# Q-Minh/point-cloud-processing

Measured on AMD Instinct MI355X. Metric: kNN+normal-estimation Mqueries/s (k=15), higher is better.
Workload: dtype f32

## Files before the change

point-cloud-processing_amd/build.py:

```python
import os
import subprocess
import sys

HERE = os.path.dirname(os.path.abspath(__file__))
CSRC = os.path.join(HERE, "csrc")
INCLUDE = os.path.join(os.path.dirname(HERE), "include")
OBJ_DIR = os.path.join(HERE, "_obj")
LIB = os.path.join(HERE, "libpcpx.so")
SOURCES = ["pcpx_query.hip", "pcpx_few.hip", "pcpx_range.hip", "pcpx_cluster.hip", "pcpx_segment.hip", "pcpx_subsample.hip", "pcpx_keypoints.hip", "pcpx_descriptors.hip", "pcpx_match.hip", "pcpx_register.hip", "pcpx_icp.hip", "pcpx_planes.hip", "pcpx_voxel.hip", "pcpx_mls.hip", "pcpx_filter.hip", "pcpx_normals.hip", "pcpx_prep.hip", "pcpx_orient.hip", "pcpx_build.hip", "pcpx_shard.hip", "pcpx_sort.hip",
           "pcpx_comm.hip", "pcpx_kd.hip", "pcpx_isosurface.hip", "pcpx_simplify.hip", "pcpx_runtime.hip", "pcpx_api.hip"]
HEADERS = [os.path.join(CSRC, "pcpx_internal.h"), os.path.join(CSRC, "pcpx_device.h"), os.path.join(CSRC, "pcpx_box_bound.h"), os.path.join(CSRC, "pcpx_eig3.h"), os.path.join(CSRC, "pcpx_curve.h"),
           os.path.join(CSRC, "pcpx_curve_table.h"), os.path.join(CSRC, "pcpx_scan.h"), os.path.join(CSRC, "pcpx_unionfind.h"), os.path.join(CSRC, "pcpx_labels.h"), os.path.join(CSRC, "pcpx_keep.h"), os.path.join(CSRC, "pcpx_stage.h"), os.path.join(CSRC, "pcpx_lease.h"), os.path.join(CSRC, "pcpx_horn.h"), os.path.join(CSRC, "pcpx_plane_solve.h"), os.path.join(CSRC, "pcpx_ransac.h"), os.path.join(CSRC, "pcpx_fixed_sum.h"), os.path.join(CSRC, "pcpx_plane_fit.h"),
           os.path.join(INCLUDE, "pcpx.h"), os.path.join(INCLUDE, "pcpx_radius.h"), os.path.join(INCLUDE, "pcpx_cluster.h"),
           os.path.join(INCLUDE, "pcpx_subsample.h"), os.path.join(INCLUDE, "pcpx_segment.h"), os.path.join(INCLUDE, "pcpx_features.h"),
           os.path.join(INCLUDE, "pcpx_keypoints.h"), os.path.join(INCLUDE, "pcpx_descriptors.h"), os.path.join(INCLUDE, "pcpx_match.h"),
           os.path.join(INCLUDE, "pcpx_register.h"), os.path.join(INCLUDE, "pcpx_icp.h"), os.path.join(INCLUDE, "pcpx_planes.h"), os.path.join(INCLUDE, "pcpx_voxel.h"), os.path.join(INCLUDE, "pcpx_mls.h")]
ARCH = "gfx950"
FLAGS = ["-O3", "-std=c++17", "-fPIC", "-ffp-contract=off", "-fno-slp-vectorize", "--offload-arch=" + ARCH,
         "-Wall", "-Werror=uninitialized", "-Werror=inline-asm", "-I" + INCLUDE]


def _hipcc():
    for c in (os.environ.get("HIPCC"), "/opt/rocm/bin/hipcc", "hipcc"):
        if c and (os.path.isabs(c) and os.path.exists(c) or not os.path.isabs(c)):
            return c
    return "hipcc"


def _stale(target, deps):
    if not os.path.exists(target):
        return True
    t = os.path.getmtime(target)
    return any(os.path.getmtime(d) > t for d in deps)


def build(force=False, verbose=False, extra_flags=(), tag=""):
    obj_dir = OBJ_DIR + ("_" + tag if tag else "")
    lib = LIB if not tag else os.path.join(HERE, "libpcpx_%s.so" % tag)
    os.makedirs(obj_dir, exist_ok=True)
    objs = []
    hipcc = _hipcc()
    for src in SOURCES:
        s = os.path.join(CSRC, src)
        o = os.path.join(obj_dir, src.replace(".hip", ".o"))
        objs.append(o)
        if force or _stale(o, [s] + HEADERS):
            cmd = [hipcc] + FLAGS + list(extra_flags) + ["-c", s, "-o", o]
            if verbose:
                print(" ".join(cmd), flush=True)
            subprocess.check_call(cmd)
    if force or _stale(lib, objs):
        cmd = [hipcc, "--offload-arch=" + ARCH, "-shared", "-fPIC", "-o", lib] + objs + ["-ldl", "-Wl,-rpath,/opt/rocm/lib"]
        if verbose:
            print(" ".join(cmd), flush=True)
        subprocess.check_call(cmd)
    return lib


if __name__ == "__main__":
    print(build(force="--force" in sys.argv, verbose=True))
```

point-cloud-processing_amd/csrc/pcpx_box_bound.h:

```cpp
#ifndef PCPX_BOX_BOUND_H
#define PCPX_BOX_BOUND_H

#include <cfloat>
#include <cmath>

#if defined(__HIPCC__)
#define PCPX_BOX_BOUND_FN __host__ __device__ inline __attribute__((always_inline))
#else
#define PCPX_BOX_BOUND_FN inline
#endif

namespace pcpx {

template <class Box>
PCPX_BOX_BOUND_FN float box_bound_fused(const Box& b, float qx, float qy, float qz)
{
    const float dx = fmaxf(fmaxf(b.lo(0) - qx, qx - b.hi(0)), 0.f);
    const float dy = fmaxf(fmaxf(b.lo(1) - qy, qy - b.hi(1)), 0.f);
    const float dz = fmaxf(fmaxf(b.lo(2) - qz, qz - b.hi(2)), 0.f);
    return __builtin_fmaf(dz, dz, __builtin_fmaf(dy, dy, __builtin_fmaf(dx, dx, b.poison)));
}

constexpr float BOX_BOUND_K = 1.f + 0x1p-20f;

PCPX_BOX_BOUND_FN float box_bound_tau(float tau) { return tau * BOX_BOUND_K + FLT_MIN; }

}

#undef PCPX_BOX_BOUND_FN
#endif
```

point-cloud-processing_amd/csrc/pcpx_device.h:

```cpp
#ifndef PCPX_DEVICE_H
#define PCPX_DEVICE_H

#include "pcpx_internal.h"

#include <cmath>
#include <limits>
#include <type_traits>

#pragma clang fp contract(off)

namespace pcpx {
namespace {

constexpr int WAVES_PER_BLOCK = 1;

__device__ __forceinline__ u32 wave_in_block() { return __builtin_amdgcn_readfirstlane(threadIdx.x >> 6); }

__device__ __forceinline__ u32 virtual_block()
{
    u32 per = gridDim.x >> 3;
    return (blockIdx.x & 7u) * per + (blockIdx.x >> 3);
}

__device__ __forceinline__ float sq3(float dx, float dy, float dz) { return dx * dx + dy * dy + dz * dz; }

typedef float float_pair __attribute__((ext_vector_type(2)));
__device__ __forceinline__ float box_d2(const NodeBox& b, float qx, float qy, float qz)
{
    float dx = fmaxf(fmaxf(b.lo(0) - qx, qx - b.hi(0)), 0.f);
    float dy = fmaxf(fmaxf(b.lo(1) - qy, qy - b.hi(1)), 0.f);
    float dz = fmaxf(fmaxf(b.lo(2) - qz, qz - b.hi(2)), 0.f);
    return sq3(dx, dy, dz) + b.poison;
}

struct NodeBox4 {
    NodeBox c[W];
};

struct Normals8 {
    float x[LEAF];
    float y[LEAF];
    float z[LEAF];
};
static_assert(sizeof(Normals8) == 12 * LEAF, "normal record must be dense");

__device__ __forceinline__ NodeBox4 load_node4(const NodeBox* first_child)
{
    typedef u32 u32x16 __attribute__((ext_vector_type(16)));
    u32x16 a, b;
    const u64 address = reinterpret_cast<uintptr_t>(first_child);
    const u32 address_lo = __builtin_amdgcn_readfirstlane(static_cast<u32>(address));
    const u32 address_hi = __builtin_amdgcn_readfirstlane(static_cast<u32>(address >> 32));
    const u64 uniform = (static_cast<u64>(address_hi) << 32) | address_lo;
    asm volatile("s_load_dwordx16 %0, %2, 0x0\n\ts_load_dwordx16 %1, %2, 0x40\n\ts_waitcnt lgkmcnt(0)"
                 : "=&s"(a), "=&s"(b)
                 : "s"(uniform));
    NodeBox4 out;
    u32* o = reinterpret_cast<u32*>(&out);
#pragma unroll
    for (int i = 0; i < 16; ++i) {
        o[i] = a[i];
        o[16 + i] = b[i];
    }
    return out;
}

__host__ __device__ __forceinline__ u32 fmix32(u32 x)
{
    x ^= x >> 16;
    x *= 0x85EBCA6Bu;
    x ^= x >> 13;
    x *= 0xC2B2AE35u;
    x ^= x >> 16;
    return x;
}

__device__ __forceinline__ bool any_lane(bool c) { return __builtin_amdgcn_ballot_w64(c) != 0ull; }

template <class T>
__device__ __forceinline__ T load_const(const T* p)
{
    static_assert(sizeof(T) % 4 == 0, "record size");
    typedef const __attribute__((address_space(4))) u32* const_u32_ptr;
    const_u32_ptr c = (const_u32_ptr)(reinterpret_cast<uintptr_t>(p));
    T out;
    u32* o = reinterpret_cast<u32*>(&out);
#pragma unroll
    for (unsigned i = 0; i < sizeof(T) / 4; ++i) o[i] = c[i];
    return out;
}

__device__ __forceinline__ u32 lds_address(const void* p)
{
    return static_cast<u32>(reinterpret_cast<uintptr_t>(p));
}


template <bool X16, bool KEEP = false>
struct WalkerT {
    u64 pend;
    u32 ploc;
    int l;
    u32 l2;
    u32 lshift0;
    u64 leaf_need[W];

    static __device__ __forceinline__ u32 level_base(int d) { return 0x55555555u >> (32 - 2 * d); }

    template <class Need>
    __device__ __forceinline__ u32 child_mask(const TreeView& t, int d, u32 loc, Need&& need)
    {
        return child_mask_at(t, level_base(d + 1) + (loc << LOGW), need);
    }
    template <class Need>
    __device__ __forceinline__ u32 child_mask_at(const TreeView& t, u32 first_child, Need&& need)
    {
        const NodeBox4 cb = X16 ? load_node4(t.nodes + first_child) : load_const(reinterpret_cast<const NodeBox4*>(t.nodes + first_child));
        u32 m;
#pragma unroll
        for (int c = W - 1; c >= 0; --c) {
            const u64 lanes = __builtin_amdgcn_ballot_w64(need(cb.c[c]));
            if (KEEP) leaf_need[c] = lanes;
            if (c == W - 1) asm("s_cmp_lg_u64 %1, 0\n\ts_cselect_b32 %0, 1, 0" : "=s"(m) : "s"(lanes) : "scc");
            else asm("s_cmp_lg_u64 %1, 0\n\ts_addc_u32 %0, %0, %0" : "+s"(m) : "s"(lanes) : "scc");
        }
        return m;
    }

    template <class Need>
    __device__ __forceinline__ bool start(const TreeView& t, Need&& need, u32& n_expand)
    {
        pend = 0;
        ploc = 0;
        l = 0;
        l2 = 0;
        lshift0 = static_cast<u32>(30 - 2 * t.depth);
        asm("" : "+s"(lshift0));
        if (t.nleaves == 0) return false;
        const NodeBox root = load_const(t.nodes);
        if (!any_lane(need(root))) return false;
        if (t.depth == 0) return true;
        ++n_expand;
        l = t.depth - 1;
        l2 = __builtin_amdgcn_readfirstlane(2u * static_cast<u32>(l));
        pend = static_cast<u64>(child_mask(t, 0, 0u, need)) << (W * l);
        return false;
    }

    __device__ __forceinline__ bool done() const { return pend == 0; }
    __device__ __forceinline__ int pop(u32& loc)
    {
        int bit;
        asm("s_ff1_i32_b64 %0, %1\n\ts_bitset0_b64 %1, %0" : "=&s"(bit), "+s"(pend));
        const int h = bit >> LOGW;
        loc = ((ploc >> (LOGW * (h - l))) << LOGW) + (static_cast<u32>(bit) & (W - 1u));
        return h;
    }
    __device__ __forceinline__ void at_leaf(u32 loc)
    {
        ploc = loc >> LOGW;
        l = 0;
        l2 = 0;
    }
    template <class Need>
    __device__ __forceinline__ void expand(const TreeView& t, int h, u32 loc, Need&& need)
    {
        l = h - 1;
        l2 = 2u * static_cast<u32>(l);
        ploc = loc;
        pend |= static_cast<u64>(child_mask(t, t.depth - h, loc, need)) << (W * l);
    }

    template <class Need>
    __device__ __forceinline__ u32 leaves_of(const TreeView& t, u32 loc, Need&& need)
    {
        l = 0;
        l2 = 0;
        ploc = loc;
        return child_mask(t, t.depth - 1, loc, need);
    }

    __device__ __forceinline__ u32 pop_scaled(u32& loc)
    {
        u32 bit;
        asm("s_ff1_i32_b64 %0, %1\n\ts_bitset0_b64 %1, %0" : "=&s"(bit), "+s"(pend));
        const u32 h4 = bit & ~(W - 1u);
        const u32 up = ploc >> ((h4 >> 1) - l2);
        asm("s_lshl2_add_u32 %0, %1, %2" : "=s"(loc) : "s"(up), "s"(bit & (W - 1u)) : "scc");
        static_assert(LOGW == 2, "s_lshl2_add_u32");
        return h4;
    }
    template <class Need>
    __device__ __forceinline__ u32 expand_any(const TreeView& t, u32 h4, u32 loc, Need&& need)
    {
        const u32 h2 = h4 >> 1;
        const u32 base = 0x55555555u >> (lshift0 + h2);
        u32 first_child;
        asm("s_lshl2_add_u32 %0, %1, %2" : "=s"(first_child) : "s"(loc), "s"(base) : "scc");
        const u32 m = child_mask_at(t, first_child, need);
        l = static_cast<int>(h4 >> LOGW) - 1;
        l2 = h2 - 2u;
        ploc = loc;
        u32 direct = m;
        if (h4 != W) {
            u64 pushed;
            asm("s_lshl_b64 %[t], %[m], %[sh]\n\ts_or_b64 %[p], %[p], %[t]" : [p] "+s"(pend), [t] "=&s"(pushed) : [m] "s"(static_cast<u64>(m)), [sh] "s"(h4 - W) : "scc");
            direct = 0;
        }
        return direct;
    }

    template <class Need>
    __device__ __forceinline__ bool next(const TreeView& t, Need&& need, u32& leaf, u32& n_expand)
    {
        while (pend != 0) {
            const int bit = __builtin_ctzll(pend);
            pend &= ~(1ull << bit);
            const int h = bit >> LOGW;
            const u32 loc = ((ploc >> (LOGW * (h - l))) << LOGW) + (static_cast<u32>(bit) & (W - 1u));
            if (h == 0) {
                ploc = loc >> LOGW;
                l = 0;
                l2 = 0;
                leaf = loc;
                return true;
            }
            ++n_expand;
            l = h - 1;
            l2 = 2u * static_cast<u32>(l);
            ploc = loc;
            pend |= static_cast<u64>(child_mask(t, t.depth - h, loc, need)) << (W * l);
        }
        return false;
    }
};
using Walker = WalkerT<true, false>;

template <bool KEEP, bool BOUNDED = false, class Need, class LeafFn>
__device__ __forceinline__ void walk_needed_leaves(const TreeView& t, Need&& need, LeafFn&& leaf_fn, const u32 leaf_end = 0u)
{
    WalkerT<true, KEEP> wk;
    u32 nexp = 0;
    if (wk.start(t, need, nexp) && t.nleaves != 0u && (!BOUNDED || leaf_end != 0u))
        leaf_fn(0u, t.leaves, ~0ull, static_cast<u32>(GROUP));
    while (!wk.done()) {
        u32 loc;
        const int h = wk.pop(loc);
        if (BOUNDED && (static_cast<u64>(loc) << (LOGW * h)) >= leaf_end) break;
        if (h > 1) {
            wk.expand(t, h, loc, need);
        } else {
            const u32 needed = wk.leaves_of(t, loc, need);
            const Leaf* records = t.leaves + (loc << LOGW);
#pragma unroll
            for (int c = 0; c < W; ++c) {
                if ((needed >> c) & 1u) {
                    u32 how_many = GROUP;
                    if (KEEP) asm("s_bcnt1_i32_b64 %0, %1" : "=s"(how_many) : "s"(wk.leaf_need[c]) : "scc");
                    const u32 leaf = (loc << LOGW) + c;
                    if (!BOUNDED || leaf < leaf_end) leaf_fn(leaf, records + c, KEEP ? wk.leaf_need[c] : ~0ull, how_many);
                }
            }
        }
    }
}

struct LaneQuery {
    float x, y, z;
    u32 row;
};
template <bool SELF>
__device__ __forceinline__ LaneQuery lane_query(const TreeView& t, const QueryView& qv, const u32 p)
{
    if (SELF) {
        const Leaf& lf = t.leaves[p / LEAF];
        return LaneQuery{lf.x[p % LEAF], lf.y[p % LEAF], lf.z[p % LEAF], lf.id[p % LEAF]};
    }
    return LaneQuery{qv.qx[p], qv.qy[p], qv.qz[p], qv.row[p]};
}

inline u32 grid_for_groups(u64 groups)
{
    u64 blocks = (groups + WAVES_PER_BLOCK - 1) / WAVES_PER_BLOCK;
    blocks = (blocks + 7) / 8 * 8;
    return static_cast<u32>(blocks);
}

inline float sanitize_eps(float eps) { return eps > 0.f ? eps : 0.f; }

}
}

#endif
```

point-cloud-processing_amd/csrc/pcpx_query.hip:

```cpp
#include "pcpx_box_bound.h"
#include "pcpx_device.h"
#include "pcpx_eig3.h"

namespace pcpx {

namespace {

constexpr size_t STATS_EXTRA = 16 + 5 * 65536 - 8;
constexpr u64 PAD_KEY = 0x7F800000FFFFFFFFull;

__device__ __forceinline__ u64 pad_key_here()
{
    u32 lo = static_cast<u32>(PAD_KEY), hi = static_cast<u32>(PAD_KEY >> 32);
    asm volatile("" : "+v"(lo), "+v"(hi));
    return (static_cast<u64>(hi) << 32) | lo;
}

__device__ __forceinline__ void ce(u64& a, u64& b)
{
    double x = __longlong_as_double(static_cast<long long>(a)), y = __longlong_as_double(static_cast<long long>(b));
    double lo, hi;
    asm("v_min_f64 %0, %1, %2" : "=v"(lo) : "v"(x), "v"(y));
    asm("v_max_f64 %0, %1, %2" : "=v"(hi) : "v"(x), "v"(y));
    a = static_cast<u64>(__double_as_longlong(lo));
// ... 308 lines not shown
template <int KCAP>
__device__ __forceinline__ float wave_radius_cap(float tau, bool valid, u32 lane)
{
    const float inf = std::numeric_limits<float>::infinity();
    asm volatile("" : "+v"(lane));
    const bool sample = (lane & 3u) == 1u;
    const float x = (valid && tau < inf) ? tau : inf;
    const u64 finite = __builtin_amdgcn_ballot_w64(sample && x < inf);
    const u32 nfinite = static_cast<u32>(__builtin_popcountll(finite));
    if (nfinite == 0) {
        const u64 any = __builtin_amdgcn_ballot_w64(x < inf);
        if (any == 0) return inf;
        return __uint_as_float(__builtin_amdgcn_readlane(__float_as_uint(x), static_cast<u32>(__builtin_ctzll(any)))) * cap_mult<KCAP>();
    }
    u32 rank = 0;
#pragma unroll
    for (u32 l = 1; l < 64; l += 4) {
        const float other = __uint_as_float(__builtin_amdgcn_readlane(__float_as_uint(x), l));
        rank += (other < x || (other == x && l < lane)) ? 1u : 0u;
    }
    const u64 is_med = __builtin_amdgcn_ballot_w64(sample && x < inf && rank == nfinite / 2);
    const float med = __uint_as_float(__builtin_amdgcn_readlane(__float_as_uint(x), static_cast<u32>(__builtin_ctzll(is_med))));
    return med * cap_mult<KCAP>();
}

struct MultiPass {
    const u64* lo = nullptr;
    u64* lo_out = nullptr;
    u64* keys = nullptr;
    u32 stride = 0;
    u32 offset = 0;
    u32 slot0 = 0;
};

struct KnnArgs {
    TreeView t;
    QueryView qv;
    u32 group_first, group_end, k;
    float eps, eps_thr;
    KnnOutputs o;
    MultiPass mp;
    u32* queue;
    unsigned long long* stats;
    KnnSchedule sch;
    u32* queue_clear;
};
typedef const __attribute__((address_space(4))) KnnArgs* knn_args_ptr;
__device__ __forceinline__ knn_args_ptr knn_args_here()
{
    u64 a = reinterpret_cast<u64>(__builtin_amdgcn_kernarg_segment_ptr());
    u32 lo = static_cast<u32>(a), hi = static_cast<u32>(a >> 32);
    asm volatile("" : "+s"(lo), "+s"(hi));
    return reinterpret_cast<knn_args_ptr>((static_cast<u64>(hi) << 32) | lo);
}
template <class T>
__device__ __forceinline__ T cold(const __attribute__((address_space(4))) T* field)
{
    static_assert(sizeof(T) % 4 == 0, "dwords");
    T out;
    u32* o = reinterpret_cast<u32*>(&out);
    const __attribute__((address_space(4))) u32* c = reinterpret_cast<const __attribute__((address_space(4))) u32*>(field);
#pragma unroll
    for (unsigned i = 0; i < sizeof(T) / 4; ++i) o[i] = c[i];
    return out;
}

template <int KCAP, bool SELF, int DIAG, bool MULTI, bool EPS_EACH, int NZ>
__device__ __forceinline__ void knn_group(const TreeView& tree, const u32 g, const float eps, const float eps_thr,
                                          unsigned long long* __restrict__ stats, u64* __restrict__ col, float* __restrict__ pub, const u32 lane,
                                          const u32 slot, const u32 part)
{
    constexpr bool STATS = DIAG == 1, COST = DIAG == 2;
    constexpr int BUF = buf_rows(KCAP);
    TreeView t = tree;
    asm volatile("" : "+s"(t.depth), "+s"(t.nodes));
    __builtin_amdgcn_s_setprio(PRIO_BASE);
    const knn_args_ptr ka = knn_args_here();
    const u32 k_arg = ka->k;
    const u32 pos_lo = ka->o.pos_lo, pos_hi = ka->o.pos_hi;
    MultiPass mp;
    if (MULTI) mp = cold(&ka->mp);
    const float* const known_d2 = STATS ? cold(&ka->o.d2) : nullptr;
    u32 k_here = k_arg;
    asm volatile("" : "+s"(k_here));
    const u32 k = k_here;
    u32 st_leaves = 0, st_expand = 0, st_compact = 0, st_app = 0, st_round2 = 0, st_seed_compact = 0, st_seed_app = 0, st_sparse = 0, st_owners = 0;
    u32 st_steps = 0;
    unsigned long long tc_walk = 0, tc_compact = 0, tc_leaf = 0, tc0 = 0, tc_mark = 0, tc_later_mark = 0;
    u32 st_later_lanes = 0;
    if (STATS) tc0 = __builtin_amdgcn_s_memtime();
    u32 tick0 = 0;
    if (!MULTI && DIAG == 0) tick0 = static_cast<u32>(__builtin_amdgcn_s_memtime());

    u32 p_here = g * GROUP + lane;
    asm volatile("" : "+v"(p_here));
    const u32 p = p_here;
    const u32 nq = SELF ? t.n : ka->qv.nq;
    const bool mine_of_part = ((p >> 3) & 7u) + 1u == part;
    const bool valid = p < nq && (!SELF || p - pos_lo < pos_hi - pos_lo) && (part == 0u || mine_of_part);
    float qx = 0.f, qy = 0.f, qz = 0.f;
    if (valid) {
        if (SELF) {
            const Leaf& lf = t.leaves[p / LEAF];
            qx = lf.x[p % LEAF];
            qy = lf.y[p % LEAF];
            qz = lf.z[p % LEAF];
        } else {
            qx = cold(&ka->qv.qx)[p];
            qy = cold(&ka->qv.qy)[p];
            qz = cold(&ka->qv.qz)[p];
        }
    }
    bool searching = valid;
    if (!SELF) {
        const bool q_nan = !(qx == qx && qy == qy && qz == qz);
        searching = valid && !q_nan;
        qx = q_nan ? 0.f : qx;
        qy = q_nan ? 0.f : qy;
        qz = q_nan ? 0.f : qz;
    }
    asm volatile("" : "+v"(qx), "+v"(qy), "+v"(qz));
    u64 lo_key = 0;
    bool has_lo = false;
    if (MULTI && mp.lo && valid) {
        lo_key = mp.lo[p - mp.slot0];
        has_lo = true;
    }
    u64 best[KCAP];
#pragma unroll
    for (int j = 0; j < KCAP; ++j) best[j] = (j < KCAP - static_cast<int>(k)) ? 0ull : PAD_KEY;
    const float inf = std::numeric_limits<float>::infinity();
    float tau = searching ? inf : -1.f;
    float tau_slack = box_bound_tau(tau);
    float tau_known = inf;
    if (STATS && known_d2 && valid && SELF) tau_known = known_d2[static_cast<u64>(t.leaves[p / LEAF].id[p % LEAF]) * k + (k - 1)];
    bool active = searching;
    int cnt = 0;
    const u32 col_addr = lds_address(col);
    u32 wa = col_addr;
    const u32 lds_row0 = __builtin_amdgcn_readfirstlane(col_addr) - 8u * __builtin_amdgcn_readfirstlane(lane);
    const u32 wa_full = lds_row0 + (static_cast<u32>(BUF - LEAF + 1) << 9);
    const u32 wa_end = lds_row0 + (static_cast<u32>(BUF) << 9);
    constexpr int packed_free = KCAP <= 16 ? PACKED_FREE16 : 0;
    const u32 wa_packed_full = packed_free > 0 ? lds_row0 + (static_cast<u32>(BUF - packed_free + 1) << 9) : wa_full;

    auto need = [&](const NodeBox& b) { return box_bound_fused(b, qx, qy, qz) <= tau_slack; };
    const EpsFilter eps_filter{deferred_eps(MULTI, EPS_EACH), eps_thr, eps, qx, qy, qz, t.leaves};

    u32 s0, s1;
    if (SELF) s0 = g * LEAVES_PER_GROUP;
    else s0 = load_const(cold(&ka->qv.seed) + g);
    s1 = s0 + LEAVES_PER_GROUP < t.nleaves ? s0 + LEAVES_PER_GROUP : t.nleaves;
    if (s0 > s1) s0 = s1;
    constexpr u32 seed_extra = KCAP <= 8 ? 0u : KCAP <= 16 ? 2u : 4u;
    if (seed_extra > 0) {
        s0 = s0 > seed_extra ? s0 - seed_extra : 0u;
        s1 = s1 + seed_extra < t.nleaves ? s1 + seed_extra : t.nleaves;
    }

    float cap = inf;
    float lo_d2 = -1.f;
    constexpr bool fast = exec_masked_accept(MULTI);

    constexpr bool packed_keys_counted_at_folds = STATS && pack_rows(MULTI, KCAP) > 0 && !EPS_EACH;
    constexpr bool count_at_accept = STATS && !packed_keys_counted_at_folds;
    auto fold = [&](bool in_seed_phase) {
        if (STATS) tc_mark = __builtin_amdgcn_s_memtime();
        if (fast) cnt = static_cast<int>((wa - col_addr) >> 9);
        if (STATS && packed_keys_counted_at_folds) st_app += static_cast<u32>(cnt);
        __builtin_amdgcn_s_setprio(PRIO_FOLD);
        if (chunked_compaction(MULTI)) compact_by8<KCAP, BUF, NZ>(best, col, cnt, eps_filter);
        else compact<KCAP, BUF>(best, col, cnt);
        __builtin_amdgcn_s_setprio(PRIO_BASE);
        float nt = __uint_as_float(static_cast<u32>(best[KCAP - 1] >> 32));
        tau = active ? fminf(nt, cap) : -1.f;
        if (STATS) tau = fminf(tau, tau_known);
        tau_slack = box_bound_tau(tau);
        wa = col_addr + (static_cast<u32>(cnt) << 9);
        if (COST) ++st_compact;
        if (STATS) {
            ++st_compact;
            if (in_seed_phase) ++st_seed_compact;
            asm volatile("" ::"v"(tau));
            tc_compact += __builtin_amdgcn_s_memtime() - tc_mark;
        }
    };
    auto fold_if_needed = [&](bool before_leaf, bool in_seed_phase) {
        if (!fast) wa = col_addr + (static_cast<u32>(cnt) << 9);
        if (any_lane(wa >= (before_leaf ? wa_full : lds_row0 + 512u))) fold(in_seed_phase);
    };

    auto candidates = [&](const u32 leaf, const bool shell) {
        if (COST) ++st_leaves;
        if (STATS) {
            ++st_leaves;
            tc_mark = __builtin_amdgcn_s_memtime();
        }
        const Leaf lf = load_const(t.leaves + leaf);
        const u32 posbase = leaf * LEAF;
        if (fast && eps_filter.on && !shell && !STATS) {
            u32 posv = posbase;
            const u64 saved = save_exec();
            static_assert(LEAF == 8, "two statements of four candidates");
            append4_if_within(lf.x, lf.y, lf.z, qx, qy, qz, tau, posv, wa, saved);
            append4_if_within(lf.x + 4, lf.y + 4, lf.z + 4, qx, qy, qz, tau, posv, wa, saved);
        } else if (fast && eps_filter.on && !shell) {
            u32 posv = posbase;
            const u64 saved = save_exec();
#pragma unroll
            for (int j = 0; j < LEAF; ++j) {
                float dx = lf.x[j] - qx, dy = lf.y[j] - qy, dz = lf.z[j] - qz;
                float d2 = sq3(dx, dy, dz);
                if (count_at_accept) st_app += (d2 <= tau) ? 1u : 0u;
                append_if_within(d2, tau, posv, wa, saved);
            }
        } else if (fast && eps_filter.on) {
            u32 posv = posbase;
            const u64 saved = save_exec();
#pragma unroll
            for (int j = 0; j < LEAF; ++j) {
                float dx = lf.x[j] - qx, dy = lf.y[j] - qy, dz = lf.z[j] - qz;
                float d2 = sq3(dx, dy, dz);
                if (count_at_accept) st_app += (d2 <= tau && d2 > lo_d2) ? 1u : 0u;
                append_if_within_shell(d2, tau, lo_d2, posv, wa, saved);
            }
        } else if (fast && !shell) {
            u32 posv = posbase;
            const u64 saved = save_exec();
#pragma unroll
            for (int j = 0; j < LEAF; ++j) {
                float dx = lf.x[j] - qx, dy = lf.y[j] - qy, dz = lf.z[j] - qz;
                float d2 = sq3(dx, dy, dz);
                if (count_at_accept) st_app += (d2 <= tau && fmaxf(fmaxf(fabsf(dx), fabsf(dy)), fabsf(dz)) >= eps) ? 1u : 0u;
                append_if(d2, tau, dx, dy, dz, eps, posv, wa, saved);
            }
        } else if (fast) {
            u32 posv = posbase;
            const u64 saved = save_exec();
#pragma unroll
            for (int j = 0; j < LEAF; ++j) {
                float dx = lf.x[j] - qx, dy = lf.y[j] - qy, dz = lf.z[j] - qz;
                float d2 = sq3(dx, dy, dz);
                if (count_at_accept) st_app += (d2 <= tau && d2 > lo_d2 && fmaxf(fmaxf(fabsf(dx), fabsf(dy)), fabsf(dz)) >= eps) ? 1u : 0u;
                append_if_shell(d2, tau, lo_d2, dx, dy, dz, eps, posv, wa, saved);
            }
        } else {
#pragma unroll
            for (int j = 0; j < LEAF; ++j) {
                float dx = lf.x[j] - qx, dy = lf.y[j] - qy, dz = lf.z[j] - qz;
                float d2 = sq3(dx, dy, dz);
                float m = fmaxf(fmaxf(fabsf(dx), fabsf(dy)), fabsf(dz));
                const u64 key = (static_cast<u64>(__float_as_uint(d2)) << 32) | (posbase + j);
                float m2 = d2 <= tau ? m : -1.f;
                bool acc = m2 >= eps && d2 > lo_d2;
                if (MULTI) acc = acc && (!has_lo || key > lo_key);
                int slot = acc ? cnt : BUF;
                col[slot * 64] = key;
                cnt += acc ? 1 : 0;
                if (count_at_accept) st_app += acc ? 1u : 0u;
            }
        }
        if (STATS) {
            asm volatile("" ::"v"(wa), "v"(cnt));
            tc_leaf += __builtin_amdgcn_s_memtime() - tc_mark;
        }
    };

    constexpr bool direct_seeds = KCAP <= SEED_DIRECT && chunked_compaction(MULTI) && !EPS_EACH && !STATS;
    auto seed_direct = [&](const u32 leaf) {
        const Leaf lf = load_const(t.leaves + leaf);
        const u32 posbase = leaf * LEAF;
        u64 nw[LEAF];
        float qx_here = qx;
#pragma unroll
        for (int j = 0; j < LEAF; ++j) {
            float dx = lf.x[j] - qx_here, dy = lf.y[j] - qy, dz = lf.z[j] - qz;
            nw[j] = (static_cast<u64>(__float_as_uint(sq3(dx, dy, dz))) << 32) | (posbase + j);
            asm volatile("" : "+v"(qx_here));
        }
        sort_network<LEAF>(nw);
        if (eps_filter.on) drop_eps_box<LEAF, LEAF>(nw, col, eps_filter);
#pragma unroll
        for (int j = 0; j < LEAF; ++j) best[KCAP - 1 - j] = key_min(best[KCAP - 1 - j], nw[j]);
        bitonic_merge<KCAP, NZ, LEAF>(best);
        tau = active ? fminf(__uint_as_float(static_cast<u32>(best[KCAP - 1] >> 32)), cap) : -1.f;
        tau_slack = box_bound_tau(tau);
    };
    for (u32 leaf = s0;; ++leaf) {
        const bool more = leaf < s1;
        if (direct_seeds && more && leaf + 1u != t.nleaves) {
            seed_direct(leaf);
            continue;
        }
        fold_if_needed(more, true);
        if (!more) break;
        candidates(leaf, false);
    }
    if (STATS) st_seed_app = st_app;
    cap = wave_radius_cap<KCAP>(tau, SELF ? valid : active, lane);
    tau = active ? fminf(tau, cap) : -1.f;
    tau_slack = box_bound_tau(tau);

    constexpr bool packed_leaves = pack_rows(MULTI, KCAP) > 0 && fast && !EPS_EACH;
    WalkerT<(KCAP > 8), packed_leaves> wk;
    auto packed_leaf = [&](const u32 leaf, const u64 who, const u32 how_many) -> u64 {
        float4* const pub_q = reinterpret_cast<float4*>(pub);
        u32* const pub_wa = reinterpret_cast<u32*>(pub) + 4 * PACKED_LEAVES;
        __builtin_amdgcn_s_setprio(PRIO_PACKED);
        u32 lane_here = lane;
        asm volatile("" : "+v"(lane_here));
        const u32 j = lane_here & 7u, i = lane_here >> 3;
        const float* rec = reinterpret_cast<const float*>(t.leaves + leaf);
        float cx = rec[j], cy = rec[LEAF + j], cz = rec[2 * LEAF + j];
        const u32 posj = leaf * LEAF + j;
        const u32 r = __builtin_amdgcn_mbcnt_hi(static_cast<u32>(who >> 32), __builtin_amdgcn_mbcnt_lo(static_cast<u32>(who), 0u));
        const bool mine = __builtin_amdgcn_inverse_ballot_w64(who);
        if (mine) {
            pub_q[r] = make_float4(qx, qy, qz, tau);
            pub_wa[r] = wa;
        }
        __builtin_amdgcn_wave_barrier();
        const u64 saved = save_exec();
        u32 s = 0;
        do {
            const float4 q = pub_q[s + i];
            asm volatile("" : "+v"(cx), "+v"(cy), "+v"(cz));
            const float dx = cx - q.x, dy = cy - q.y, dz = cz - q.z;
            const float d2 = sq3(dx, dy, dz);
            const u32 slot = lds_address(pub_wa + s + i);
            u32 at, inside;
            if (packed_free > 0)
                asm volatile("v_cmpx_le_f32_e32 %[d2], %[tau]\n\t"
                             "v_mov_b32_e32 %[at], 0x200\n\t"
                             "ds_add_rtn_u32 %[at], %[slot], %[at]\n\t"
                             "s_waitcnt lgkmcnt(0)\n\t"
                             "v_subrev_u32_e32 %[m], %[end], %[at]\n\t"
                             "v_ashrrev_i32_e32 %[m], 31, %[m]\n\t"
                             "v_bfi_b32 %[at], %[m], %[at], %[spare]\n\t"
                             "ds_write2_b32 %[at], %[pos], %[d2] offset1:1\n\t"
                             "s_mov_b64 exec, %[saved]"
                             : [at] "=&v"(at), [m] "=&v"(inside)
                             : [d2] "v"(d2), [tau] "v"(q.w), [slot] "v"(slot), [end] "s"(wa_end), [spare] "s"(wa_end + 480u), [pos] "v"(posj), [saved] "s"(saved)
                             : "vcc", "memory");
            else
                asm volatile("v_cmpx_le_f32_e32 %[d2], %[tau]\n\t"
                             "v_mov_b32_e32 %[at], 0x200\n\t"
                             "ds_add_rtn_u32 %[at], %[slot], %[at]\n\t"
                             "s_waitcnt lgkmcnt(0)\n\t"
                             "ds_write2_b32 %[at], %[pos], %[d2] offset1:1\n\t"
                             "s_mov_b64 exec, %[saved]"
                             : [at] "=&v"(at)
                             : [d2] "v"(d2), [tau] "v"(q.w), [slot] "v"(slot), [pos] "v"(posj), [saved] "s"(saved)
                             : "vcc", "memory");
            s += 8u;
        } while (s < how_many);
        __builtin_amdgcn_wave_barrier();
        u32 now = wa;
        if (mine) {
            now = pub_wa[r];
            reinterpret_cast<float*>(pub_q + r)[3] = -1.f;
        }
        __builtin_amdgcn_wave_barrier();
        __builtin_amdgcn_s_setprio(PRIO_BASE);
        if (packed_free == 0) {
            wa = now;
            return 0ull;
        }
        const bool lost_keys = now > col_addr + (static_cast<u32>(BUF) << 9);
        wa = lost_keys ? wa : now;
        return __builtin_amdgcn_ballot_w64(lost_keys);
    };
    auto packed_take_back = [&](const u64 lost) {
        if (__builtin_amdgcn_inverse_ballot_w64(lost)) {
            const u32 column_end = col_addr + (static_cast<u32>(BUF) << 9);
            const u64 pad = pad_key_here();
            for (u32 a = wa; a < column_end; a += 512u) asm volatile("ds_write_b64 %0, %1" ::"v"(a), "v"(pad) : "memory");
        }
    };
    const u32 seed_count = s1 - s0;
    u32 packed_limit = packed_leaves ? PACKED_LEAVES : 0;
    for (u32 rounds = 0;;) {
        const u32 packed_limit_now = __builtin_amdgcn_readfirstlane(packed_limit);
        bool root_leaf = wk.start(t, need, st_expand);
        (void)root_leaf;
        if (STATS) tc_mark = __builtin_amdgcn_s_memtime();
        u32 direct = 0, direct_node = 0;
        for (;;) {
            if (direct == 0) {
                if (wk.done()) break;
                const u32 h4 = wk.pop_scaled(direct_node);
                ++st_expand;
                direct = wk.expand_any(t, h4, direct_node, need);
            }
            while (direct != 0) {
                u32 loc, child;
                asm("s_ff1_i32_b32 %0, %1\n\ts_bitset0_b32 %1, %0\n\ts_lshl2_add_u32 %2, %3, %0" : "=&s"(child), "+s"(direct), "=s"(loc) : "s"(direct_node) : "scc");
                if (loc - s0 >= seed_count) {
                    if (STATS) tc_walk += __builtin_amdgcn_s_memtime() - tc_mark;
                    if (!packed_leaves) {
                        fold_if_needed(true, false);
                        candidates(loc, rounds != 0u);
                    } else {
                        const u32 c = child;
                        u64 who, upper;
                        u32 how_many, packed_form, full_from;
                        asm("s_bitcmp1_b32 %[c], 0\n\ts_cselect_b64 %[w], %[n1], %[n0]\n\ts_cselect_b64 %[u], %[n3], %[n2]\n\t"
                            "s_bitcmp1_b32 %[c], 1\n\ts_cselect_b64 %[w], %[u], %[w]\n\t"
                            "s_bcnt1_i32_b64 %[m], %[w]\n\t"
                            "s_cmp_le_u32 %[m], %[lim]\n\ts_cselect_b32 %[pf], 1, 0\n\ts_cselect_b32 %[thr], %[tp], %[td]"
                            : [w] "=&s"(who), [u] "=&s"(upper), [m] "=&s"(how_many), [pf] "=&s"(packed_form), [thr] "=&s"(full_from)
                            : [c] "s"(c), [n0] "s"(wk.leaf_need[0]), [n1] "s"(wk.leaf_need[1]), [n2] "s"(wk.leaf_need[2]), [n3] "s"(wk.leaf_need[3]),
                              [lim] "s"(packed_limit_now), [tp] "s"(wa_packed_full), [td] "s"(wa_full)
                            : "scc");
                        u64 todo = who;
                        for (;;) {
                            if ((__builtin_amdgcn_ballot_w64(wa >= full_from) & todo) != 0) fold(false);
                            if (packed_form == 0u) break;
                            if (STATS) tc_mark = __builtin_amdgcn_s_memtime();
                            todo = packed_leaf(loc, todo, how_many);
                            if (COST) st_steps += (how_many + 7u) >> 3;
                            if (STATS) {
                                asm volatile("" ::"v"(wa));
                                tc_leaf += __builtin_amdgcn_s_memtime() - tc_mark;
                            }
                            if (__builtin_expect(todo == 0, 1)) break;
                            packed_take_back(todo);
                            how_many = static_cast<u32>(__builtin_popcountll(todo));
                            full_from = 0u;
                        }
                        if (packed_form != 0u) {
                            if (COST) ++st_sparse;
                            if (STATS) ++st_leaves, ++st_sparse, st_owners += how_many;
                        } else {
                            candidates(loc, rounds != 0u);
                        }
                    }
                    if (STATS) tc_mark = __builtin_amdgcn_s_memtime();
                }
            }
        }
        if (STATS) tc_walk += __builtin_amdgcn_s_memtime() - tc_mark;
        fold_if_needed(false, false);
        if (!(cap < inf)) break;
        const float kth = __uint_as_float(static_cast<u32>(best[KCAP - 1] >> 32));
        const bool failed = active && !(kth <= cap);
        if (!any_lane(failed)) break;
        if (COST) ++st_round2, st_later_lanes += static_cast<u32>(__builtin_popcountll(__builtin_amdgcn_ballot_w64(failed)));
        if (STATS) {
            ++st_round2;
            if (tc_later_mark == 0) tc_later_mark = __builtin_amdgcn_s_memtime();
            st_later_lanes += static_cast<u32>(__builtin_popcountll(__builtin_amdgcn_ballot_w64(failed)));
        }
        lo_d2 = cap;
        const NodeBox root = load_const(t.nodes);
        const float ex = root.hi(0) - root.lo(0), ey = root.hi(1) - root.lo(1), ez = root.hi(2) - root.lo(2);
        const float diag2 = sq3(ex, ey, ez);
        const float grown = cap * CAP_GROW;
        ++rounds;
        packed_limit = 0;
        cap = (grown > cap && grown < diag2 * 4.f && rounds < 12u) ? grown : inf;
        active = failed;
        tau = active ? fminf(kth, cap) : -1.f;
        tau_slack = box_bound_tau(tau);
        cnt = 0;
        wa = col_addr;
    }

    if (STATS) {
        u32 app = st_app, sapp = st_seed_app;
#pragma unroll
        for (int off = 32; off > 0; off >>= 1) {
            app += __shfl_xor(app, off);
            sapp += __shfl_xor(sapp, off);
        }
        if (lane == 0) {
            atomicAdd(&stats[0], static_cast<unsigned long long>(st_leaves));
            atomicAdd(&stats[1], static_cast<unsigned long long>(st_expand));
            atomicAdd(&stats[2], static_cast<unsigned long long>(st_compact));
            atomicAdd(&stats[12], static_cast<unsigned long long>(st_seed_compact));
            atomicAdd(&stats[13], static_cast<unsigned long long>(sapp));
            atomicAdd(&stats[14], static_cast<unsigned long long>(st_sparse));
            atomicAdd(&stats[15], static_cast<unsigned long long>(st_owners));
            atomicAdd(&stats[3], static_cast<unsigned long long>(app));
            atomicAdd(&stats[4], 1ull);
            atomicAdd(&stats[5], static_cast<unsigned long long>(s1 - s0));
            atomicAdd(&stats[6], static_cast<unsigned long long>(st_round2));
            atomicAdd(&stats[7], tc_walk);
            atomicAdd(&stats[8], tc_compact);
            atomicAdd(&stats[9], tc_leaf);
            atomicAdd(&stats[10], static_cast<unsigned long long>(__builtin_amdgcn_s_memtime()) - tc0);
            if (tc_later_mark != 0) atomicAdd(&stats[STATS_EXTRA], static_cast<unsigned long long>(__builtin_amdgcn_s_memtime()) - tc_later_mark);
            atomicAdd(&stats[STATS_EXTRA + 1], static_cast<unsigned long long>(st_later_lanes));
        }
    }

    if (!MULTI && DIAG == 0) {
        const knn_args_ptr kt = knn_args_here();
        u32* const gtime = cold(&kt->sch.gtime);
        if (gtime) {
            const u32 ticks = (static_cast<u32>(__builtin_amdgcn_s_memtime()) - tick0) >> 6;
            u32 lane_again = lane;
            asm volatile("" : "+v"(lane_again));
            if (lane_again == 0) gtime[g - kt->group_first] = ticks;
        }
    }
    if (COST) {
        u32* const events = cold(&knn_args_here()->sch.events);
        if (lane == 0) {
            uint4 e;
            e.x = st_expand, e.y = (st_leaves & 0xFFFFFFu) | (st_round2 << 24), e.z = (st_sparse & 0xFFFFFu) | ((st_later_lanes < 0xFFFu ? st_later_lanes : 0xFFFu) << 20),
            e.w = (st_compact << 16) | (st_steps < 0xFFFFu ? st_steps : 0xFFFFu);
            reinterpret_cast<uint4*>(events)[slot] = e;
        }
    }
    const int first_slot = KCAP - static_cast<int>(k);
    if (!SELF) {
        const knn_args_ptr kq = knn_args_here();
        u32 pq = g * GROUP + lane;
        asm volatile("" : "+v"(pq));
        float x = 0.f, y = 0.f, z = 0.f;
        if (valid) {
            x = cold(&kq->qv.qx)[pq];
            y = cold(&kq->qv.qy)[pq];
            z = cold(&kq->qv.qz)[pq];
        }
        u32 kill = (x == x && y == y && z == z) ? 0u : ~0u;
        asm volatile("" : "+v"(kill));
#pragma unroll
        for (int s = NZ; s < KCAP; ++s) {
            const u32 lo = static_cast<u32>(best[s]) | kill;
            const u32 hi = (static_cast<u32>(best[s] >> 32) & ~kill) | (static_cast<u32>(PAD_KEY >> 32) & kill);
            best[s] = (static_cast<u64>(hi) << 32) | lo;
        }
    }
    if (MULTI) {
        const MultiPass mp = cold(&knn_args_here()->mp);
        if (valid) {
            u64* dst = mp.keys + static_cast<u64>(p - mp.slot0) * mp.stride + mp.offset;
#pragma unroll
            for (int s = 0; s < KCAP; ++s) {
                int j = s - first_slot;
                if (j >= 0) dst[j] = best[s];
            }
            mp.lo_out[p - mp.slot0] = best[KCAP - 1];
        }
        return;
    }
    u32* const pos_col = reinterpret_cast<u32*>(col);
    auto pos_slot = [&](int s) -> u32& { return pos_col[(s >> 1) * 128 + (s & 1)]; };
#pragma unroll
    for (int s = NZ; s < KCAP; ++s) {
        u64 key = best[s];
        bool real = s >= first_slot && key != PAD_KEY;
        u32 ps = real ? static_cast<u32>(key) : 0u;
        pos_slot(s) = ps;
        u32 id = t.leaves[ps / LEAF].id[ps % LEAF];
        asm volatile("" : "+v"(id));
        best[s] = real ? ((key & 0xFFFFFFFF00000000ull) | id) : key;
    }
    bool unordered = false;
#pragma unroll
    for (int s = 0; s + 1 < KCAP; ++s) unordered |= best[s] > best[s + 1];
    for (int round = 0; round < KCAP && any_lane(unordered); ++round) {
#pragma unroll
        for (int parity = 0; parity < 2; ++parity) {
#pragma unroll
            for (int s = parity; s + 1 < KCAP; s += 2) {
                const bool sw = best[s] > best[s + 1];
                const u64 a = sw ? best[s + 1] : best[s], b = sw ? best[s] : best[s + 1];
                best[s] = a;
                best[s + 1] = b;
                if (sw) {
                    const u32 pa = pos_slot(s), pb = pos_slot(s + 1);
                    pos_slot(s) = pb;
                    pos_slot(s + 1) = pa;
                }
            }
        }
        unordered = false;
#pragma unroll
        for (int s = 0; s + 1 < KCAP; ++s) unordered |= best[s] > best[s + 1];
    }
    auto restore_column = [&]() {
        const u64 pad = pad_key_here();
#pragma unroll
        for (int r = 0; r < (KCAP + 1) / 2; ++r) col[r * 64] = pad;
    };

    if (!valid) {
        restore_column();
        return;
    }
    u32 g_again = g;
    asm volatile("" : "+s"(g_again));
    u32 p_row = g_again * GROUP + lane;
    asm volatile("" : "+v"(p_row));
    const knn_args_ptr kb = knn_args_here();
    const KnnOutputs o = cold(&kb->o);
    u32 row = SELF ? t.leaves[p_row / LEAF].id[p_row % LEAF] : cold(&kb->qv.row)[p_row];
    if (SELF && o.by_position) row = p_row + o.pos_bias;
    if (SELF && o.tau) o.tau[p_row] = key_d2(best[KCAP - 1]);
    u32 found = 0;
    u32 okmask = 0;
    const u32 stride = o.row_stride ? o.row_stride : k;
    const u64 ob = static_cast<u64>(row) * stride;
    const bool whole_rows = stride == static_cast<u32>(KCAP) && first_slot == NZ && !STATS;
    auto store_whole_rows = [&](auto FS) {
        constexpr int fs = decltype(FS)::value;
#pragma unroll
        for (int c = 0; c < KCAP / 4; ++c) {
            u32 id4[4];
            float d4[4];
#pragma unroll
            for (int e = 0; e < 4; ++e) {
                const int sl = 4 * c + e + fs;
                const u64 key = sl < KCAP ? best[sl < KCAP ? sl : 0] : PAD_KEY;
                const bool ok = key != PAD_KEY;
                id4[e] = ok ? static_cast<u32>(key) : INVALID_ID;
                d4[e] = __uint_as_float(static_cast<u32>(key >> 32));
            }
            if (o.idx) *reinterpret_cast<uint4*>(o.idx + ob + 4 * c) = make_uint4(id4[0], id4[1], id4[2], id4[3]);
            if (o.d2) *reinterpret_cast<float4*>(o.d2 + ob + 4 * c) = make_float4(d4[0], d4[1], d4[2], d4[3]);
        }
    };
    if (whole_rows) store_whole_rows(std::integral_constant<int, NZ>{});
#pragma unroll
    for (int s = NZ; s < KCAP; ++s) {
        int j = s - first_slot;
        if (j >= 0) {
            u64 key = best[s];
            bool ok = key != PAD_KEY;
            if (!whole_rows) {
                if (o.idx) o.idx[ob + j] = ok ? static_cast<u32>(key) : INVALID_ID;
                if (o.d2 && !STATS) o.d2[ob + j] = __uint_as_float(static_cast<u32>(key >> 32));
            }
            found += ok ? 1u : 0u;
            okmask |= ok ? (1u << s) : 0u;
        }
    }
    if (!whole_rows) {
        for (u32 j = k; j < stride; ++j) {
            if (o.idx) o.idx[ob + j] = INVALID_ID;
            if (o.d2 && !STATS) o.d2[ob + j] = __uint_as_float(static_cast<u32>(PAD_KEY >> 32));
        }
    }
    if (o.cnt) o.cnt[row] = found;

    if (o.meandist) {
        float sum = 0.f;
#pragma unroll
        for (int s = NZ; s < KCAP; ++s) {
            bool ok = (okmask >> s) & 1u;
            float d = sqrtf(__uint_as_float(static_cast<u32>(best[s] >> 32)));
            sum += ok ? d : 0.f;
        }
        o.meandist[row] = sum / static_cast<float>(found);
    }

    if (o.normals || o.centroids || (SELF && o.nc4)) {
        float nbx[KCAP], nby[KCAP], nbz[KCAP];
#pragma unroll
        for (int s = NZ; s < KCAP; ++s) {
            const u32 ps = pos_slot(s);
            const Leaf& lf = t.leaves[ps / LEAF];
            nbx[s] = lf.x[ps % LEAF];
            nby[s] = lf.y[ps % LEAF];
            nbz[s] = lf.z[ps % LEAF];
        }
        float sx = 0.f, sy = 0.f, sz = 0.f;
#pragma unroll
        for (int s = NZ; s < KCAP; ++s) {
            bool ok = (okmask >> s) & 1u;
            sx += ok ? nbx[s] : 0.f;
            sy += ok ? nby[s] : 0.f;
            sz += ok ? nbz[s] : 0.f;
        }
        float fn = static_cast<float>(found);
        float mx = sx / fn, my = sy / fn, mz = sz / fn;
        if (o.centroids) {
            o.centroids[3ull * row] = mx;
            o.centroids[3ull * row + 1] = my;
            o.centroids[3ull * row + 2] = mz;
        }
        if (!o.normals && !(SELF && o.nc4)) {
            restore_column();
            return;
        }
// ... 540 lines not shown
```

Before: 2895.

## Start self-query tree walk from the group's own path instead of the root

For self queries, the tree walk no longer descends from the root. Each lane of the wave instead loads one sibling node along the query group's root-to-leaf path, and the walker's pending set is seeded with the siblings whose box gap to the group's own leaf box is within the wave radius cap. The aim is to skip the repeated top-down expansions and their dependent node loads at the start of every walk round. It adds a per-round vector load of path nodes and a coarser box-to-box pruning test, which may admit more subtrees than per-query tests would.

After: 3015 (median of 6 runs). 1.04x the previous value.

```diff
diff --git a/point-cloud-processing_amd/build.py b/point-cloud-processing_amd/build.py
--- a/point-cloud-processing_amd/build.py
+++ b/point-cloud-processing_amd/build.py
@@ -9,7 +9,7 @@
 LIB = os.path.join(HERE, "libpcpx.so")
 SOURCES = ["pcpx_query.hip", "pcpx_few.hip", "pcpx_range.hip", "pcpx_cluster.hip", "pcpx_segment.hip", "pcpx_subsample.hip", "pcpx_keypoints.hip", "pcpx_descriptors.hip", "pcpx_match.hip", "pcpx_register.hip", "pcpx_icp.hip", "pcpx_planes.hip", "pcpx_voxel.hip", "pcpx_mls.hip", "pcpx_filter.hip", "pcpx_normals.hip", "pcpx_prep.hip", "pcpx_orient.hip", "pcpx_build.hip", "pcpx_shard.hip", "pcpx_sort.hip",
            "pcpx_comm.hip", "pcpx_kd.hip", "pcpx_isosurface.hip", "pcpx_simplify.hip", "pcpx_runtime.hip", "pcpx_api.hip"]
-HEADERS = [os.path.join(CSRC, "pcpx_internal.h"), os.path.join(CSRC, "pcpx_device.h"), os.path.join(CSRC, "pcpx_box_bound.h"), os.path.join(CSRC, "pcpx_eig3.h"), os.path.join(CSRC, "pcpx_curve.h"),
+HEADERS = [os.path.join(CSRC, "pcpx_internal.h"), os.path.join(CSRC, "pcpx_device.h"), os.path.join(CSRC, "pcpx_box_bound.h"), os.path.join(CSRC, "pcpx_path_start.h"), os.path.join(CSRC, "pcpx_eig3.h"), os.path.join(CSRC, "pcpx_curve.h"),
            os.path.join(CSRC, "pcpx_curve_table.h"), os.path.join(CSRC, "pcpx_scan.h"), os.path.join(CSRC, "pcpx_unionfind.h"), os.path.join(CSRC, "pcpx_labels.h"), os.path.join(CSRC, "pcpx_keep.h"), os.path.join(CSRC, "pcpx_stage.h"), os.path.join(CSRC, "pcpx_lease.h"), os.path.join(CSRC, "pcpx_horn.h"), os.path.join(CSRC, "pcpx_plane_solve.h"), os.path.join(CSRC, "pcpx_ransac.h"), os.path.join(CSRC, "pcpx_fixed_sum.h"), os.path.join(CSRC, "pcpx_plane_fit.h"),
            os.path.join(INCLUDE, "pcpx.h"), os.path.join(INCLUDE, "pcpx_radius.h"), os.path.join(INCLUDE, "pcpx_cluster.h"),
            os.path.join(INCLUDE, "pcpx_subsample.h"), os.path.join(INCLUDE, "pcpx_segment.h"), os.path.join(INCLUDE, "pcpx_features.h"),
diff --git a/point-cloud-processing_amd/csrc/pcpx_box_bound.h b/point-cloud-processing_amd/csrc/pcpx_box_bound.h
--- a/point-cloud-processing_amd/csrc/pcpx_box_bound.h
+++ b/point-cloud-processing_amd/csrc/pcpx_box_bound.h
@@ -25,6 +25,15 @@
 
 PCPX_BOX_BOUND_FN float box_bound_tau(float tau) { return tau * BOX_BOUND_K + FLT_MIN; }
 
+template <class Box, class QueryBox>
+PCPX_BOX_BOUND_FN float box_gap_bound_fused(const Box& u, const QueryBox& w)
+{
+    const float gx = fmaxf(fmaxf(u.lo(0) - w.hi(0), w.lo(0) - u.hi(0)), 0.f);
+    const float gy = fmaxf(fmaxf(u.lo(1) - w.hi(1), w.lo(1) - u.hi(1)), 0.f);
+    const float gz = fmaxf(fmaxf(u.lo(2) - w.hi(2), w.lo(2) - u.hi(2)), 0.f);
+    return __builtin_fmaf(gz, gz, __builtin_fmaf(gy, gy, __builtin_fmaf(gx, gx, u.poison)));
+}
+
 }
 
 #undef PCPX_BOX_BOUND_FN
diff --git a/point-cloud-processing_amd/csrc/pcpx_device.h b/point-cloud-processing_amd/csrc/pcpx_device.h
--- a/point-cloud-processing_amd/csrc/pcpx_device.h
+++ b/point-cloud-processing_amd/csrc/pcpx_device.h
@@ -2,6 +2,8 @@
 #define PCPX_DEVICE_H
 
 #include "pcpx_internal.h"
+#include "pcpx_box_bound.h"
+#include "pcpx_path_start.h"
 
 #include <cmath>
 #include <limits>
@@ -95,6 +97,12 @@
     return static_cast<u32>(reinterpret_cast<uintptr_t>(p));
 }
 
+
+struct QueryBox {
+    float lo3[3], hi3[3];
+    __device__ float lo(int a) const { return lo3[a]; }
+    __device__ float hi(int a) const { return hi3[a]; }
+};
 
 template <bool X16, bool KEEP = false>
 struct WalkerT {
@@ -145,6 +153,47 @@
         l2 = __builtin_amdgcn_readfirstlane(2u * static_cast<u32>(l));
         pend = static_cast<u64>(child_mask(t, 0, 0u, need)) << (W * l);
         return false;
+    }
+
+    struct PathBoxes {
+        NodeBox mine;
+        NodeBox own[2];
+        u64 lanes;
+    };
+    static __device__ __forceinline__ PathBoxes path_fetch(const TreeView& t, const u32 g, u32 lane)
+    {
+        asm volatile("" : "+v"(lane));
+        const u32 depth = static_cast<u32>(t.depth);
+        const PathLane pl = path_lane(lane, g, depth, 30u - 2u * depth);
+        PathBoxes pb;
+        pb.lanes = __builtin_amdgcn_ballot_w64(pl.on);
+        typedef float f32x4 __attribute__((ext_vector_type(4)));
+        typedef const __attribute__((address_space(1))) f32x4* global_f32x4_ptr;
+        const global_f32x4_ptr mine = (global_f32x4_ptr)(reinterpret_cast<uintptr_t>(t.nodes + pl.node));
+        const f32x4 a = mine[0], b = mine[1];
+        pb.mine.set(a.x, a.y, a.z, a.w, b.x, b.y);
+        pb.mine.poison = b.z;
+        pb.mine.pad = 0.f;
+        const u32 own0 = depth != 0u ? level_base(t.depth - 1) + 2u * g : 0u;
+        pb.own[0] = load_const(t.nodes + own0);
+        pb.own[1] = load_const(t.nodes + own0 + (depth != 0u ? 1u : 0u));
+        return pb;
+    }
+    __device__ __forceinline__ void start_path(const TreeView& t, const u32 g, const PathBoxes& pb, const float cap)
+    {
+        lshift0 = static_cast<u32>(30 - 2 * t.depth);
+        asm("" : "+s"(lshift0));
+        ploc = g >> 1;
+        l = 1;
+        l2 = 2;
+        QueryBox w;
+        const bool two = __float_as_uint(pb.own[1].poison) == 0u;
+#pragma unroll
+        for (int a = 0; a < 3; ++a) {
+            w.lo3[a] = two ? fminf(pb.own[0].lo(a), pb.own[1].lo(a)) : pb.own[0].lo(a);
+            w.hi3[a] = two ? fmaxf(pb.own[0].hi(a), pb.own[1].hi(a)) : pb.own[0].hi(a);
+        }
+        pend = __builtin_amdgcn_ballot_w64(box_gap_bound_fused(pb.mine, w) <= box_bound_tau(cap)) & pb.lanes;
     }
 
     __device__ __forceinline__ bool done() const { return pend == 0; }
diff --git a/point-cloud-processing_amd/csrc/pcpx_path_start.h b/point-cloud-processing_amd/csrc/pcpx_path_start.h
--- /dev/null
+++ b/point-cloud-processing_amd/csrc/pcpx_path_start.h
@@ -0,0 +1,37 @@
+#ifndef PCPX_PATH_START_H
+#define PCPX_PATH_START_H
+
+#include <cstdint>
+
+#if defined(__HIPCC__)
+#define PCPX_PATH_START_FN __host__ __device__ inline __attribute__((always_inline))
+#else
+#define PCPX_PATH_START_FN inline
+#endif
+
+namespace pcpx {
+
+struct PathLane {
+    bool on;
+    std::uint32_t node;
+};
+
+PCPX_PATH_START_FN PathLane path_lane(std::uint32_t lane, std::uint32_t g, std::uint32_t depth, std::uint32_t level_shift0)
+{
+    const std::uint32_t h = lane >> 2, c = lane & 3u;
+    const bool stands = h >= 1u && h < depth;
+    const std::uint32_t hc = stands ? h : 1u;
+    const std::uint32_t local = ((g >> (2u * hc - 1u)) << 2) + c;
+    const std::uint32_t pair = hc == 1u ? 1u : 0u;
+    const bool own = (local >> pair) == ((2u * g) >> (2u * hc - 2u + pair));
+    const std::uint32_t base = 0x55555555u >> ((level_shift0 + 2u + 2u * hc) & 31u);
+    PathLane out;
+    out.on = stands && !own;
+    out.node = out.on ? base + local : 0u;
+    return out;
+}
+
+}
+
+#undef PCPX_PATH_START_FN
+#endif
diff --git a/point-cloud-processing_amd/csrc/pcpx_query.hip b/point-cloud-processing_amd/csrc/pcpx_query.hip
--- a/point-cloud-processing_amd/csrc/pcpx_query.hip
+++ b/point-cloud-processing_amd/csrc/pcpx_query.hip
@@ -634,7 +634,8 @@
     tau_slack = box_bound_tau(tau);
 
     constexpr bool packed_leaves = pack_rows(MULTI, KCAP) > 0 && fast && !EPS_EACH;
-    WalkerT<(KCAP > 8), packed_leaves> wk;
+    using WalkerK = WalkerT<(KCAP > 8), packed_leaves>;
+    WalkerK wk;
     auto packed_leaf = [&](const u32 leaf, const u64 who, const u32 how_many) -> u64 {
         float4* const pub_q = reinterpret_cast<float4*>(pub);
         u32* const pub_wa = reinterpret_cast<u32*>(pub) + 4 * PACKED_LEAVES;
@@ -713,8 +714,13 @@
     u32 packed_limit = packed_leaves ? PACKED_LEAVES : 0;
     for (u32 rounds = 0;;) {
         const u32 packed_limit_now = __builtin_amdgcn_readfirstlane(packed_limit);
-        bool root_leaf = wk.start(t, need, st_expand);
-        (void)root_leaf;
+        if (SELF) {
+            wk.start_path(t, g, WalkerK::path_fetch(t, g, lane), cap);
+            ++st_expand;
+        } else {
+            bool root_leaf = wk.start(t, need, st_expand);
+            (void)root_leaf;
+        }
         if (STATS) tc_mark = __builtin_amdgcn_s_memtime();
         u32 direct = 0, direct_node = 0;
         for (;;) {
```
